# facebookresearch/iSDF

Measured on NVIDIA H100. Metric: train ray-samples/sec, higher is better.
Workload: dtype bf16x3 (bf16 hi/lo split, fp32 accumulate; weight-gradient operands single bf16)

## Files before the change

include/isdf_b200.h:

```cpp
#ifndef ISDF_B200_H_
#define ISDF_B200_H_

#include <stdint.h>

#ifdef __cplusplus
extern "C" {
#endif

typedef struct isdfb_ctx isdfb_ctx;

typedef enum {
  ISDFB_OK = 0,
  ISDFB_ERR_ARG = -1,
  ISDFB_ERR_CUDA = -2,
  ISDFB_ERR_CAPACITY = -3,
  ISDFB_ERR_STATE = -4
} isdfb_status;

typedef enum {
  ISDFB_PREC_FP32 = 0,
  ISDFB_PREC_BF16X3 = 1,
  ISDFB_PREC_BF16 = 2,
  ISDFB_PREC_BF16X3G = 3
} isdfb_precision;
// ... 24 lines not shown
} isdfb_loss_cfg;

typedef struct { float fx, fy, cx, cy; int32_t H, W; } isdfb_camera;

int isdfb_create(const isdfb_model_cfg* cfg, int device, isdfb_ctx** out);
int isdfb_destroy(isdfb_ctx* ctx);
const char* isdfb_last_error(const isdfb_ctx* ctx);
int64_t isdfb_param_count(const isdfb_ctx* ctx);
int32_t isdfb_embedding_size(const isdfb_ctx* ctx);
int64_t isdfb_launch_count(const isdfb_ctx* ctx);

int isdfb_pack_weights(isdfb_ctx* ctx, const float* params_flat, void* stream);

int isdfb_gather_rays(isdfb_ctx* ctx, const float* depth, const float* normals,
                      const int64_t* frame_map, int32_t normals_use_frame_map,
                      const int64_t* ib, const int64_t* ih, const int64_t* iw, int64_t n_rays,
                      const isdfb_camera* cam, float* depth_out, float* normal_out,
                      uint8_t* valid_out, void* stream);
int isdfb_sample_rays(isdfb_ctx* ctx, const float* T_WC , const int64_t* frame_map,
                      const int64_t* ib, const int64_t* ih, const int64_t* iw,
                      const float* dirs_C_in, const float* depth_sample, const float* far,
                      const float* near, const float* u_strat, const float* n_near,
                      const float* lin, int64_t n_rays, int32_t n_strat, int32_t n_surf,
                      const isdfb_camera* cam, float min_depth, float dist_behind,
                      float* pc , float* z_vals , float* dirs_C ,
                      float* T_WC_sample , void* stream);

int isdfb_sample_fused(isdfb_ctx* ctx, const float* depth, const float* normals, const float* T_WC,
                       const int64_t* frame_map, int32_t normals_use_frame_map, int32_t n_frames,
                       int32_t n_rays_per_frame, int32_t n_strat, int32_t n_surf, const isdfb_camera* cam,
                       float min_depth, float dist_behind, const float* lin, uint64_t seed, int64_t* ib, int64_t* ih,
                       int64_t* iw, float* pc, float* z_vals, float* dirs_C, float* T_WC_sample, float* depth_sample,
                       float* norm_sample, uint8_t* ray_valid, float* noise, float* inv_count, void* stream);

int isdfb_select_window(isdfb_ctx* ctx, const float* frame_avg_losses , int32_t n_frames,
                        int32_t window_size, uint64_t seed, int64_t* frame_map , void* stream);

int isdfb_ingest_normals(isdfb_ctx* ctx, const float* depth, const isdfb_camera* cam, float* normals,
                         void* stream);

int isdfb_pe_encode(isdfb_ctx* ctx, const float* x, int64_t n, float* out, void* stream);

int isdfb_mlp_forward(isdfb_ctx* ctx, const float* x, const float* noise, float noise_std,
                      int64_t n, float* sdf, void* stream);
int isdfb_mlp_forward_grad(isdfb_ctx* ctx, const float* x, const float* noise, float noise_std,
                           int64_t n, float* sdf, float* grad, void* stream);

int isdfb_mlp_forward_grid(isdfb_ctx* ctx, const float* lin , int32_t dim,
                           const float* scale , const float* transform ,
                           float* sdf , void* stream);

int isdfb_bounds_pc(isdfb_ctx* ctx, const float* pc, const float* z_vals, const float* depth_sample,
                    const uint8_t* ray_valid, int64_t n_rays, int32_t n_samples, float* bounds,
                    float* grad_vec, void* stream);

int isdfb_train_fwd_bwd(isdfb_ctx* ctx, const float* pc, const float* z_vals,
                        const float* depth_sample, const float* dirs_C, const float* T_WC_sample,
                        const float* norm_sample, const float* noise, const uint8_t* ray_valid,
                        int64_t n_rays, int32_t n_samples, const isdfb_loss_cfg* loss,
                        float* sdf, float* grad, float* loss_mat, float* loss_sums, void* stream);
int isdfb_zero_grad(isdfb_ctx* ctx, void* stream);
int isdfb_export_grads(isdfb_ctx* ctx, float* grads_flat, void* stream);

int isdfb_frame_bins(isdfb_ctx* ctx, const float* loss_mat, const uint8_t* ray_valid,
                     const int64_t* ib, const int64_t* ih, const int64_t* iw, int64_t n_rays,
                     int32_t n_samples, int32_t n_frames, int32_t H, int32_t W, int32_t factor,
                     float* loss_approx, float* frame_avg, void* stream);

int isdfb_step_finish(isdfb_ctx* ctx, const float* loss_mat, const uint8_t* ray_valid,
                      const int64_t* ib, const int64_t* ih, const int64_t* iw, int64_t n_rays,
                      int32_t n_samples, int32_t n_frames, int32_t H, int32_t W, int32_t factor,
                      float* loss_approx, float* frame_avg, const int64_t* frame_map, float* frame_avg_losses,
                      float* loss_sums, const float* inv_count, float* means_out, void* stream);

int isdfb_adamw(isdfb_ctx* ctx, float* params_flat, float* m, float* v, int64_t step, double lr,
                double beta1, double beta2, double eps, double weight_decay, float grad_scale,
                void* stream);
int isdfb_adamw_graph(isdfb_ctx* ctx, float* params_flat, float* m, float* v, double lr, double beta1,
                      double beta2, double eps, double weight_decay, float grad_scale, void* stream);
int isdfb_adamw_set_step(isdfb_ctx* ctx, int64_t step, void* stream);
int isdfb_grad_buffer(isdfb_ctx* ctx, float** ptr, int64_t* n_floats);

int isdfb_set_grad_exchange(isdfb_ctx* ctx, float* local0, float* local1, float* mcast0, float* mcast1,
                            int64_t n_floats);
int isdfb_select_grad_buffer(isdfb_ctx* ctx, int32_t which);
int isdfb_zero_grad_buffer(isdfb_ctx* ctx, int32_t which, void* stream);

int isdfb_mesh_count(isdfb_ctx* ctx, const float* sdf, int32_t dim, int64_t* n_verts ,
                     int64_t* n_faces , void* stream);
int isdfb_mesh_emit(isdfb_ctx* ctx, const float* sdf, int32_t dim, const float* scale ,
                    const float* transform , float* verts, int64_t cap_verts, int32_t* faces,
                    int64_t cap_faces, void* stream);

int isdfb_mesh_cloud(isdfb_ctx* ctx, const float* depth, const float* T_WC, int32_t n_frames, int32_t H, int32_t W,
                     int32_t H_vis, int32_t W_vis, float fx, float fy, float cx, float cy, float* cloud, float* box,
                     void* stream);
int isdfb_mesh_crop_count(isdfb_ctx* ctx, const float* cloud, int64_t n_cloud, float crop_dist, const float* verts,
                          int64_t n_verts, const int32_t* faces, int64_t n_faces, int64_t* n_verts_kept ,
                          int64_t* n_faces_kept , void* stream);
int isdfb_mesh_crop_emit(isdfb_ctx* ctx, const float* verts, int64_t n_verts, const int32_t* faces, int64_t n_faces,
                         float* verts_out, int64_t cap_verts, int32_t* faces_out, int64_t cap_faces, void* stream);

int isdfb_gt_sdf_sample(isdfb_ctx* ctx, const float* lattice, int32_t nx, int32_t ny, int32_t nz,
                        const double* origin , const double* spacing , const float* pts_f32,
                        const double* pts_f64, int64_t n, double fill, double* out, uint8_t* in_bounds, void* stream);

#define ISDFB_EVAL_NSTATS 17
int isdfb_sdf_error_stats(isdfb_ctx* ctx, const float* pred, const double* gt, const uint8_t* in_bounds,
                          const uint8_t* valid, int64_t n, double* out, void* stream);

int isdfb_points_visible(isdfb_ctx* ctx, const float* pts, int64_t n, const float* T_CW, const float* depth,
                         int32_t n_frames, int32_t H, int32_t W, float fx, float fy, float cx, float cy, float trunc,
                         uint8_t* vis, void* stream);

int isdfb_gt_sdf_grad(isdfb_ctx* ctx, const float* lattice, int32_t nx, int32_t ny, int32_t nz,
                      const double* origin , const double* spacing , const float* pts_f32,
                      const double* pts_f64, int64_t n, double delta, double* grad, uint8_t* valid, void* stream);

int isdfb_sdf_split_stats(isdfb_ctx* ctx, const float* pred, const double* gt, int64_t n, int64_t n_vox, double* out,
                          void* stream);

int isdfb_grad_cosdist(isdfb_ctx* ctx, const float* pred, const double* gt, const int64_t* gt_index, int64_t n,
                       double eps, double* out, void* stream);

#define ISDFB_CHOMP_MAX_EPS 4
int isdfb_chomp_costs(isdfb_ctx* ctx, const float* pred, const double* gt, const uint8_t* in_bounds, int64_t n,
                      const double* eps , int32_t n_eps, double* out, void* stream);

#define ISDFB_VOXELIZE_MAX_DEPTH 9
#define ISDFB_GT_SDF_MAX_DIM 16384
int isdfb_voxelize_count(isdfb_ctx* ctx, const double* verts, int64_t n_verts, const void* faces, int32_t faces_int64,
                         int64_t n_faces, double pitch, const double* origin , int64_t* box_lo ,
                         int64_t* box_dims , void* stream);
int isdfb_voxelize_emit(isdfb_ctx* ctx, const double* verts, int64_t n_verts, const void* faces, int32_t faces_int64,
                        int64_t n_faces, double pitch, const double* origin ,
                        const int64_t* box_lo , const int64_t* box_dims , uint8_t* box,
                        void* stream);
int isdfb_fill_holes(isdfb_ctx* ctx, uint8_t* box, int32_t nx, int32_t ny, int32_t nz, void* stream);
int isdfb_occupancy_sdf(isdfb_ctx* ctx, const uint8_t* occ, int32_t nx, int32_t ny, int32_t nz, double voxel_size,
                        double* sdf, void* stream);

int isdfb_profile_enable(isdfb_ctx* ctx, int32_t enable);
int isdfb_profile_read(isdfb_ctx* ctx, double* chain_ms, double* dw_ms, int64_t* n_chain, int64_t* n_dw);

int isdfb_debug_program(int32_t n_freqs, int32_t hidden, int32_t block, int32_t mode, int32_t* steps_out,
                        int32_t max_steps);

int isdfb_debug_mc_table(uint8_t* rows, int32_t* max_tris);

int isdfb_debug_buffers(isdfb_ctx* ctx, float** aux, int64_t* aux_stride_floats, void** dwl_hi,
                        void** dwl_lo, int64_t* dwl_stride_bytes, int32_t* n_aux, int32_t* n_dwl,
                        int64_t* tiles_cap, void** sig16);

#ifdef __cplusplus
}
#endif
#endif
```

isdf_b200/_lib.py:

```python
import ctypes as C
import os

_HERE = os.path.dirname(os.path.abspath(__file__))
LIB_PATH = os.path.join(_HERE, "lib", "libisdf_b200.so")

PREC_FP32, PREC_BF16X3, PREC_BF16, PREC_BF16X3G = 0, 1, 2, 3
PRECISIONS = {"fp32": PREC_FP32, "bf16x3": PREC_BF16X3, "bf16": PREC_BF16, "bf16x3g": PREC_BF16X3G}


class ModelCfg(C.Structure):
    _fields_ = [("n_freqs", C.c_int32), ("hidden", C.c_int32), ("block", C.c_int32),
                ("has_transform", C.c_int32), ("scale_input", C.c_float), ("scale_output", C.c_float),
                ("transform", C.c_float * 12), ("precision", C.c_int32), ("max_points", C.c_int32)]


class LossCfg(C.Structure):
    _fields_ = [("trunc_weight", C.c_float), ("trunc_distance", C.c_float), ("eik_weight", C.c_float),
                ("eik_apply_dist", C.c_float), ("grad_weight", C.c_float), ("orien_loss", C.c_int32),
                ("loss_type", C.c_int32), ("noise_std", C.c_float), ("inv_count", C.c_float),
                ("inv_count_dev", C.c_void_p), ("bounds_dev", C.c_void_p), ("grad_vec_dev", C.c_void_p)]


class Camera(C.Structure):
    _fields_ = [("fx", C.c_float), ("fy", C.c_float), ("cx", C.c_float), ("cy", C.c_float),
                ("H", C.c_int32), ("W", C.c_int32)]


P = C.c_void_p
I64 = C.c_int64
I32 = C.c_int32
F = C.c_float
D = C.c_double

SIGNATURES = {
    "isdfb_create": (C.c_int, [C.POINTER(ModelCfg), C.c_int, C.POINTER(P)]),
    "isdfb_destroy": (C.c_int, [P]),
    "isdfb_last_error": (C.c_char_p, [P]),
    "isdfb_param_count": (I64, [P]),
    "isdfb_embedding_size": (I32, [P]),
    "isdfb_launch_count": (I64, [P]),
    "isdfb_pack_weights": (C.c_int, [P, P, P]),
    "isdfb_gather_rays": (C.c_int, [P, P, P, P, I32, P, P, P, I64, C.POINTER(Camera), P, P, P, P]),
    "isdfb_sample_rays": (C.c_int, [P, P, P, P, P, P, P, P, P, P, P, P, P, I64, I32, I32, C.POINTER(Camera), F, F,
                                    P, P, P, P, P]),
    "isdfb_sample_fused": (C.c_int, [P, P, P, P, P, I32, I32, I32, I32, I32, C.POINTER(Camera), F, F, P, C.c_uint64,
                                     P, P, P, P, P, P, P, P, P, P, P, P, P]),
    "isdfb_ingest_normals": (C.c_int, [P, P, C.POINTER(Camera), P, P]),
    "isdfb_pe_encode": (C.c_int, [P, P, I64, P, P]),
    "isdfb_mlp_forward": (C.c_int, [P, P, P, F, I64, P, P]),
    "isdfb_mlp_forward_grad": (C.c_int, [P, P, P, F, I64, P, P, P]),
    "isdfb_mlp_forward_grid": (C.c_int, [P, P, I32, C.POINTER(F), C.POINTER(F), P, P]),
    "isdfb_bounds_pc": (C.c_int, [P, P, P, P, P, I64, I32, P, P, P]),
    "isdfb_train_fwd_bwd": (C.c_int, [P, P, P, P, P, P, P, P, P, I64, I32, C.POINTER(LossCfg), P, P, P, P, P]),
    "isdfb_zero_grad": (C.c_int, [P, P]),
    "isdfb_set_grad_exchange": (C.c_int, [P, P, P, P, P, I64]),
    "isdfb_select_grad_buffer": (C.c_int, [P, I32]),
    "isdfb_zero_grad_buffer": (C.c_int, [P, I32, P]),
    "isdfb_export_grads": (C.c_int, [P, P, P]),
    "isdfb_frame_bins": (C.c_int, [P, P, P, P, P, P, I64, I32, I32, I32, I32, I32, P, P, P]),
    "isdfb_step_finish": (C.c_int, [P, P, P, P, P, P, I64, I32, I32, I32, I32, I32, P, P, P, P, P, P, P, P]),
    "isdfb_select_window": (C.c_int, [P, P, I32, I32, C.c_uint64, P, P]),
    "isdfb_adamw": (C.c_int, [P, P, P, P, I64, D, D, D, D, D, F, P]),
    "isdfb_adamw_graph": (C.c_int, [P, P, P, P, D, D, D, D, D, F, P]),
    "isdfb_adamw_set_step": (C.c_int, [P, I64, P]),
    "isdfb_grad_buffer": (C.c_int, [P, C.POINTER(P), C.POINTER(I64)]),
    "isdfb_mesh_count": (C.c_int, [P, P, I32, C.POINTER(I64), C.POINTER(I64), P]),
    "isdfb_mesh_emit": (C.c_int, [P, P, I32, C.POINTER(F), C.POINTER(F), P, I64, P, I64, P]),
    "isdfb_mesh_cloud": (C.c_int, [P, P, P, I32, I32, I32, I32, I32, F, F, F, F, P, P, P]),
    "isdfb_mesh_crop_count": (C.c_int, [P, P, I64, F, P, I64, P, I64, C.POINTER(I64), C.POINTER(I64), P]),
    "isdfb_mesh_crop_emit": (C.c_int, [P, P, I64, P, I64, P, I64, P, I64, P]),
    "isdfb_gt_sdf_sample": (C.c_int, [P, P, I32, I32, I32, C.POINTER(C.c_double), C.POINTER(C.c_double), P, P, I64,
                                      C.c_double, P, P, P]),
    "isdfb_sdf_error_stats": (C.c_int, [P, P, P, P, P, I64, P, P]),
    "isdfb_points_visible": (C.c_int, [P, P, I64, P, P, I32, I32, I32, F, F, F, F, F, P, P]),
    "isdfb_gt_sdf_grad": (C.c_int, [P, P, I32, I32, I32, C.POINTER(C.c_double), C.POINTER(C.c_double), P, P, I64,
                                    C.c_double, P, P, P]),
    "isdfb_sdf_split_stats": (C.c_int, [P, P, P, I64, I64, P, P]),
    "isdfb_grad_cosdist": (C.c_int, [P, P, P, P, I64, C.c_double, P, P]),
    "isdfb_chomp_costs": (C.c_int, [P, P, P, P, I64, C.POINTER(C.c_double), I32, P, P]),
    "isdfb_voxelize_count": (C.c_int, [P, P, I64, P, I32, I64, D, C.POINTER(D), C.POINTER(I64), C.POINTER(I64), P]),
    "isdfb_voxelize_emit": (C.c_int, [P, P, I64, P, I32, I64, D, C.POINTER(D), C.POINTER(I64), C.POINTER(I64), P, P]),
    "isdfb_fill_holes": (C.c_int, [P, P, I32, I32, I32, P]),
    "isdfb_occupancy_sdf": (C.c_int, [P, P, I32, I32, I32, D, P, P]),
    "isdfb_profile_enable": (C.c_int, [P, I32]),
    "isdfb_profile_read": (C.c_int, [P, C.POINTER(C.c_double), C.POINTER(C.c_double), C.POINTER(I64), C.POINTER(I64)]),
    "isdfb_debug_program": (C.c_int, [I32, I32, I32, I32, C.POINTER(I32), I32]),
    "isdfb_debug_mc_table": (C.c_int, [C.POINTER(C.c_uint8), C.POINTER(I32)]),
    "isdfb_debug_buffers": (C.c_int, [P, C.POINTER(P), C.POINTER(I64), C.POINTER(P), C.POINTER(P), C.POINTER(I64),
                                      C.POINTER(I32), C.POINTER(I32), C.POINTER(I64), C.POINTER(P)]),
}

_lib = None


def load():
    global _lib
    if _lib is not None:
        return _lib
    if not os.path.exists(LIB_PATH):
        raise RuntimeError(
            "isdf_b200: CUDA library %s not found. Build it with `python -c 'import __graft_entry__ as g; "
            "g.build()'` (nvcc, sm_90a). There is no CPU fallback." % LIB_PATH)
    lib = C.CDLL(LIB_PATH)
    for name, (res, args) in SIGNATURES.items():
        fn = getattr(lib, name)
        fn.restype = res
        fn.argtypes = args
    _lib = lib
    return lib


ERR_ARG, ERR_CUDA, ERR_CAPACITY, ERR_STATE = -1, -2, -3, -4


class IsdfbError(RuntimeError):

    def __init__(self, msg, rc=None):
        super().__init__(msg)
        self.rc = rc


def check(rc, ctx=None):
    if rc != 0:
        msg = load().isdfb_last_error(ctx)
        raise IsdfbError("isdf_b200 error %d: %s" % (rc, msg.decode() if msg else "?"), rc)
```

isdf_b200/csrc/tc_dw.cu:

```cuda
#include "tc_path.cuh"

#define DW_CONS_WG 2
#define DW_THREADS (128 * (1 + DW_CONS_WG))
#define DW_CONS_REGS 224
#define DW_PROD_REGS 56

template <int kPasses> struct DwCfg {
  static constexpr int kXBytes = 4096 * (kPasses == 3 ? 2 : 1);
  static constexpr int kYBytes = 8192 * (kPasses == 3 ? 2 : 1);
  static constexpr int kStageBytes = kXBytes + kYBytes;
  static constexpr int kStages = (kPasses == 3) ? 8 : 12;
  static constexpr int kSmem = kStages * kStageBytes + 512 + 256;
};

struct DwSmemTail {
  uint64_t full[12], empty[12];
};

template <int kPasses>
__global__ void __launch_bounds__(DW_THREADS, 1) tc_dw_kernel(const __grid_constant__ TcDwArgs args) {
  using Cfg = DwCfg<kPasses>;
  extern __shared__ __align__(1024) uint8_t smem[];
  uint8_t* ring = smem;
  uint8_t* ones = smem + Cfg::kStages * Cfg::kStageBytes;
  DwSmemTail* tail = reinterpret_cast<DwSmemTail*>(ones + 512);
  const int warp = threadIdx.x >> 5, lane = threadIdx.x & 31;

  const int job_id = blockIdx.x % args.n_jobs;
  const int split = blockIdx.x / args.n_jobs;
  const int n_splits = ((int)gridDim.x - 1 - job_id) / args.n_jobs + 1;
  const int my_tiles = (args.n_tiles > split) ? (args.n_tiles - 1 - split) / n_splits + 1 : 0;
  const TcDwJob& job = args.jobs[job_id];

  if (threadIdx.x < 128) reinterpret_cast<uint32_t*>(ones)[threadIdx.x] = 0x3F803F80u;
  if (threadIdx.x == 0) {
    for (int i = 0; i < Cfg::kStages; ++i) { mbar_init(smem_u32(&tail->full[i]), 1); mbar_init(smem_u32(&tail->empty[i]), DW_CONS_WG); }
    mbar_fence_init();
  }
  fence_proxy_async_smem();
  __syncthreads();

  bool has_main = false, has_db = false, has_dw = false;
  for (int pi = 0; pi < job.n_pairs; ++pi) {
    has_main |= job.pair[pi].y_arr >= 0;
    has_db |= job.pair[pi].ones == 1;
    has_dw |= job.pair[pi].ones == 2;
  }

  if (warp < 4) {
    reg_dec<DW_PROD_REGS>();
    if (warp == 0 && elect_one()) {
      uint32_t j = 0;
      for (int it = 0; it < my_tiles; ++it) {
        const size_t tile_off = (size_t)(args.tile0 + split + it * n_splits) * TC_DWL_TILE_BYTES;
        for (int pi = 0; pi < job.n_pairs; ++pi) {
          const TcDwPair pr = job.pair[pi];
          const size_t xo = (size_t)pr.x_arr * args.dwl_stride + tile_off + (size_t)job.half * 4096;
          const size_t yo = (size_t)(pr.y_arr < 0 ? 0 : pr.y_arr) * args.dwl_stride + tile_off;
          const uint32_t bytes = Cfg::kXBytes + (pr.y_arr >= 0 ? Cfg::kYBytes : 0);
          for (int ks = 0; ks < 8; ++ks, ++j) {
            const uint32_t stage = j % Cfg::kStages, ph = (j / Cfg::kStages) & 1;
            mbar_wait(smem_u32(&tail->empty[stage]), ph ^ 1);
            const uint32_t bar = smem_u32(&tail->full[stage]);
            const uint32_t dst = smem_u32(ring + stage * Cfg::kStageBytes);
            mbar_arrive_expect_tx(bar, bytes);
            bulk_g2s(dst, args.dwl_hi + xo + (size_t)ks * 8192, 4096, bar);
            if (kPasses == 3) bulk_g2s(dst + 4096, args.dwl_lo + xo + (size_t)ks * 8192, 4096, bar);
            if (pr.y_arr >= 0) {
              bulk_g2s(dst + Cfg::kXBytes, args.dwl_hi + yo + (size_t)ks * 8192, 8192, bar);
              if (kPasses == 3) bulk_g2s(dst + Cfg::kXBytes + 8192, args.dwl_lo + yo + (size_t)ks * 8192, 8192, bar);
            }
          }
        }
      }
    }
  } else {
    reg_inc<DW_CONS_REGS>();
    const int g = (warp >> 2) - 1, wq = warp & 3, q4 = lane & 3;
    const bool leader = (threadIdx.x & 127) == 0;
    float d_main[128], d_db[8], d_dw[8];
#pragma unroll
    for (int r = 0; r < 128; ++r) d_main[r] = 0.f;
#pragma unroll
    for (int r = 0; r < 8; ++r) { d_db[r] = 0.f; d_dw[r] = 0.f; }
    uint32_t j = 0, acc_main = 0, acc_db = 0, acc_dw = 0;
    const uint64_t b_ones = gmma_desc(smem_u32(ones), 128, 256);
    wgmma_fence();
    for (int it = 0; it < my_tiles; ++it) {
      for (int pi = 0; pi < job.n_pairs; ++pi) {
        const TcDwPair pr = job.pair[pi];
#pragma unroll 1
        for (int ks = 0; ks < 8; ++ks, ++j) {
          const uint32_t stage = j % Cfg::kStages, ph = (j / Cfg::kStages) & 1;
          mbar_wait(smem_u32(&tail->full[stage]), ph);
          const uint32_t base = smem_u32(ring + stage * Cfg::kStageBytes);
          const uint64_t ah = gmma_desc(base + 2048u * g, 128, 256);
          const uint64_t al = gmma_desc(base + 4096 + 2048u * g, 128, 256);
          if (pr.y_arr >= 0) {
            const uint64_t bh = gmma_desc(base + Cfg::kXBytes, 128, 256);
            wgmma_m64n256k16<1, 1>(d_main, ah, bh, acc_main);
            if (kPasses == 3) {
              wgmma_m64n256k16<1, 1>(d_main, al, bh, 1);
              wgmma_m64n256k16<1, 1>(d_main, ah, gmma_desc(base + Cfg::kXBytes + 8192, 128, 256), 1);
            }
            acc_main = 1;
          }
          if (pr.ones == 1) {
            wgmma_m64n16k16<1, 1>(d_db, ah, b_ones, acc_db);
            if (kPasses == 3) wgmma_m64n16k16<1, 1>(d_db, al, b_ones, 1);
            acc_db = 1;
          } else if (pr.ones == 2) {
            wgmma_m64n16k16<1, 1>(d_dw, ah, b_ones, acc_dw);
            if (kPasses == 3) wgmma_m64n16k16<1, 1>(d_dw, al, b_ones, 1);
            acc_dw = 1;
          }
          wgmma_commit();
          if (j > 0) {
            wgmma_wait<1>();
            if (leader) mbar_arrive(smem_u32(&tail->empty[(j - 1) % Cfg::kStages]));
          }
        }
      }
    }
    wgmma_wait<0>();
    wgmma_fence_operands<128>(d_main);
    wgmma_fence_operands<8>(d_db);
    wgmma_fence_operands<8>(d_dw);
    if (my_tiles > 0) {
      const int r0 = job.half * 128 + 64 * g + 16 * wq + (lane >> 2);
      if (has_main) {
#pragma unroll
        for (int rh = 0; rh < 2; ++rh) {
          float* grow = args.g_packed + job.g_off + (size_t)(r0 + 8 * rh) * job.ld;
          if (job.perm_half > 0) {
#pragma unroll
            for (int i = 0; i < 32; ++i)
#pragma unroll
              for (int e = 0; e < 2; ++e) {
                const int nat = pe_nat_col(job.col0 + 8 * i + 2 * q4 + e, job.perm_half);
                if (nat < job.ld) grad_add(grow + nat, d_main[4 * i + 2 * rh + e], 0);
              }
          } else {
#pragma unroll
            for (int i = 0; i < 32; ++i) grad_add2(grow + 8 * i + 2 * q4, d_main[4 * i + 2 * rh], d_main[4 * i + 2 * rh + 1]);
          }
        }
      }
      if (q4 == 0) {
#pragma unroll
        for (int rh = 0; rh < 2; ++rh) {
          if (has_db) grad_add(args.g_packed + job.db_off + r0 + 8 * rh, d_db[2 * rh], 0);
          if (has_dw) grad_add(args.g_packed + args.wout_off + r0 + 8 * rh, args.scale_output * d_dw[2 * rh], 0);
        }
      }
    }
    if (args.g_mc) {
      __shared__ int s_last;
      const int t = threadIdx.x - 128;
      __threadfence();
      named_bar_sync(3, 128 * DW_CONS_WG);
      if (t == 0) {
        const int prev = (my_tiles > 0) ? atomicAdd(args.counters + job_id, 1) : -1;
        s_last = (prev == args.expect[job_id] - 1) ? 1 : 0;
        if (s_last) args.counters[job_id] = 0;
      }
      named_bar_sync(3, 128 * DW_CONS_WG);
      if (s_last) {
        __threadfence();
        const size_t base = job.g_off + (size_t)(job.half * 128) * job.ld;
        if (has_main) {
          float4* src = reinterpret_cast<float4*>(args.g_packed + base) + t;
          float* dst = args.g_mc_out + base + (size_t)t * 4;
#pragma unroll 1
          for (int it = 0; it < 32; it += 8) {
            float4 r[8];
#pragma unroll
            for (int u = 0; u < 8; ++u) r[u] = __ldcg(src + (size_t)(it + u) * 256);
#pragma unroll
            for (int u = 0; u < 8; ++u) {
              grad_add4(dst + (size_t)(it + u) * 1024, r[u].x, r[u].y, r[u].z, r[u].w, 1);
              __stcg(src + (size_t)(it + u) * 256, make_float4(0.f, 0.f, 0.f, 0.f));
            }
          }
        }
        if (t < 128) {
          const int row = job.half * 128 + t;
          if (has_db) {
            float* p = args.g_packed + job.db_off + row;
            grad_add(args.g_mc_out + job.db_off + row, __ldcg(p), 1);
            __stcg(p, 0.f);
          }
          if (has_dw) {
            float* p = args.g_packed + args.wout_off + row;
            grad_add(args.g_mc_out + args.wout_off + row, __ldcg(p), 1);
            __stcg(p, 0.f);
          }
        }
      }
    }
  }
}

int tc_dw_launch(isdfb_ctx* ctx, const TcDwArgs& args, int passes, int grid, cudaStream_t st) {
  if (grid < args.n_jobs)
    ISDFB_FAIL(ctx, ISDFB_ERR_ARG, "weight-gradient launch of %d CTAs for %d jobs: every job needs a CTA", grid,
               args.n_jobs);
  if (passes == 3) {
    tc_dw_kernel<3><<<grid, DW_THREADS, DwCfg<3>::kSmem, st>>>(args);
  } else {
    tc_dw_kernel<1><<<grid, DW_THREADS, DwCfg<1>::kSmem, st>>>(args);
  }
  ISDFB_LAUNCHED(ctx);
  ISDFB_CUDA_OK(ctx, cudaGetLastError());
  return ISDFB_OK;
}

int tc_dw_init(isdfb_ctx* ctx) {
  ISDFB_CUDA_OK(ctx, cudaFuncSetAttribute(tc_dw_kernel<3>, cudaFuncAttributeMaxDynamicSharedMemorySize, DwCfg<3>::kSmem));
  ISDFB_CUDA_OK(ctx, cudaFuncSetAttribute(tc_dw_kernel<1>, cudaFuncAttributeMaxDynamicSharedMemorySize, DwCfg<1>::kSmem));
  return ISDFB_OK;
}
```

isdf_b200/csrc/tc_path.cu:

```cuda
#include "tc_path.cuh"
#include <new>

static TcStep& add_step(TcChainArgs& a, int unit, int orient, int epi, int layer, int aux = 0) {
  TcStep& s = a.steps[a.n_steps++];
  s.unit = unit; s.orient = orient; s.epi = epi; s.layer = (int16_t)layer; s.aux = (int16_t)aux;
  s.addp = -1; s.flags = 0; s.peh = 0; s.eh = 0;
  return s;
}

enum { PART_CAT_S1 = 0, PART_CAT_S2 = 1, PART_CAT_S3 = 2, PART_CAT_S2_H1 = 3, PART_L0_S1 = 4, PART_L0_S3 = 5 };

static void build_program(const ModelLayout& lay, int mode, int NE, TcChainArgs& a) {
  const int L = lay.L, ic = lay.block + 1, UE = L, U0B = L + 1, UEB = L + 2;
  a.n_steps = 0;
  add_step(a, UE, 0, EPI_RAW, 0, PART_CAT_S1);
  if (NE == 2) {
    TcStep& r = add_step(a, 0, 0, EPI_RAW, 0, PART_L0_S1);
    r.flags = STF_PE_E; r.peh = 1;
    add_step(a, UEB, 0, EPI_RAW, 0, PART_CAT_S1).flags = STF_RAW_ADD;
  }
  for (int l = 0; l < L; ++l) {
    TcStep& t = add_step(a, (l == 0 && NE == 2) ? U0B : l, 0, l == L - 1 ? EPI_S1_LAST : EPI_S1, l);
    if (l == 0 && NE == 2) t.addp = PART_L0_S1;
    if (l == ic) t.addp = PART_CAT_S1;
// ... 212 lines not shown

static inline int wave1_dw_grid(const TcState* tc, int rest) {
  const int free_sms = tc->num_sms - rest;
  return free_sms > tc->dw.n_jobs ? free_sms : tc->dw.n_jobs;
}

static int tc_forward_impl(isdfb_ctx* ctx, const float* x, const float* noise, float noise_std, int64_t n, float* sdf,
                           float* grad, cudaStream_t st, const TcGrid* grid) {
  TcState* tc = reinterpret_cast<TcState*>(ctx->tc);
  for (int64_t p0 = 0; p0 < n; p0 += ctx->cap) {
    const int64_t nc = (n - p0 < ctx->cap) ? (n - p0) : ctx->cap;
    TcChainArgs a = tc->proto[grad ? TC_MODE_FWD_GRAD : TC_MODE_FWD];
    if (grid) a.grid = *grid;
    a.n_points = nc;
    a.n_tiles = (int)((nc + TC_TILE - 1) / TC_TILE);
    a.p0 = p0;
    a.x = x ? x + p0 * 3 : nullptr;
    a.noise = noise ? noise + p0 : nullptr;
    a.noise_std = noise_std;
    a.sdf_out = sdf + p0;
    a.g_out = grad ? grad + p0 * 3 : nullptr;
    const int n_cta = a.n_tiles < tc->num_sms ? a.n_tiles : tc->num_sms;
    const int pi = prof_begin(tc, st);
    int rc = tc_chain_launch(ctx, a, passes_of(ctx), n_cta, st);
    if (rc) return rc;
    prof_mark(tc, pi, 1, st);
  }
  return ISDFB_OK;
}

int tc_forward(isdfb_ctx* ctx, const float* x, const float* noise, float noise_std, int64_t n, float* sdf,
               float* grad, cudaStream_t st) {
  return tc_forward_impl(ctx, x, noise, noise_std, n, sdf, grad, st, nullptr);
}

int tc_forward_grid(isdfb_ctx* ctx, const float* lin, int dim, const float* scale, const float* transform, float* sdf,
                    cudaStream_t st) {
  if ((int64_t)dim * dim * dim >= (1LL << 32))
    ISDFB_FAIL(ctx, ISDFB_ERR_ARG, "grid dim %d too large for the tensor-core path (dim^3 must be < 2^32)", dim);
  TcGrid g;
  memset(&g, 0, sizeof(g));
  g.lin = lin; g.dim = dim;
  for (int i = 0; i < 3; ++i) g.scale[i] = scale ? scale[i] : 1.f;
  g.has_transform = transform ? 1 : 0;
  if (transform)
    for (int r = 0; r < 3; ++r) {
      for (int c = 0; c < 3; ++c) g.R[r * 3 + c] = transform[r * 4 + c];
      g.t[r] = transform[r * 4 + 3];
    }
  return tc_forward_impl(ctx, nullptr, nullptr, 0.f, (int64_t)dim * dim * dim, sdf, nullptr, st, &g);
}

int tc_train(isdfb_ctx* ctx, const float* pc, const float* z_vals, const float* depth_sample, const float* dirs_C,
             const float* T_WC_sample, const float* norm_sample, const float* noise, const uint8_t* ray_valid,
             int64_t n_rays, int32_t S, const isdfb_loss_cfg* loss, float* sdf, float* grad, float* loss_mat,
             float* loss_sums, cudaStream_t st) {
  TcState* tc = reinterpret_cast<TcState*>(ctx->tc);
  const int64_t n = n_rays * S;
  if (n >= (1LL << 32))
    ISDFB_FAIL(ctx, ISDFB_ERR_ARG, "%lld samples per step exceed the tensor-core path's 2^32", (long long)n);
  const bool two_wave_ok = !tc->profiling;
  int32_t expect[TC_MAX_JOBS] = {0};
  if (ctx->g_xchg) {
    auto plan = [&](int grid, int tiles) {
      for (int j = 0; j < tc->dw.n_jobs; ++j) {
        const int n_splits = (grid - 1 - j) / tc->dw.n_jobs + 1;
        expect[j] += n_splits < tiles ? n_splits : tiles;
      }
    };
    for (int64_t p0 = 0; p0 < n; p0 += ctx->cap) {
      const int64_t nc = (n - p0 < ctx->cap) ? (n - p0) : ctx->cap;
      const int tiles = (int)((nc + TC_TILE - 1) / TC_TILE);
      if (tiles > tc->num_sms && tiles < 2 * tc->num_sms && two_wave_ok) {
        const int rest = tiles - tc->num_sms;
        plan(wave1_dw_grid(tc, rest), tc->num_sms);
        plan(tc->num_sms, rest);
      } else {
        plan(tc->num_sms, tiles);
      }
    }
  }
  for (int64_t p0 = 0; p0 < n; p0 += ctx->cap) {
    const int64_t nc = (n - p0 < ctx->cap) ? (n - p0) : ctx->cap;
    TcChainArgs a = tc->proto[TC_MODE_TRAIN];
    a.n_points = nc;
    a.n_tiles = (int)((nc + TC_TILE - 1) / TC_TILE);
    a.p0 = p0;
    a.S = S;
    a.loss = *loss;
    a.x = pc + p0 * 3;
    a.noise = noise ? noise + p0 : nullptr;
    a.noise_std = loss->noise_std;
    a.sdf_out = sdf + p0;
    a.g_out = grad ? grad + p0 * 3 : nullptr;
    a.z_vals = z_vals; a.depth = depth_sample; a.dirs_C = dirs_C; a.T_WC = T_WC_sample; a.normals = norm_sample;
    a.ray_valid = ray_valid;
    a.loss_mat = loss_mat;
    a.loss_sums = loss_sums;
    a.g_packed = ctx->g_xchg ? ctx->g_mc[ctx->g_sel] : ctx->g_packed;
    a.g_mc = ctx->g_xchg ? 1 : 0;
    const int total_tiles = a.n_tiles;
    const int pi = prof_begin(tc, st);
    TcDwArgs d = tc->dw;
    d.g_mc = ctx->g_xchg ? 1 : 0;
    d.g_packed = ctx->g_xchg ? ctx->g_own : ctx->g_packed;
    d.g_mc_out = ctx->g_xchg ? ctx->g_mc[ctx->g_sel] : nullptr;
    d.counters = tc->dw_counters;
    for (int j = 0; j < TC_MAX_JOBS; ++j) d.expect[j] = expect[j];
    int rc;
    if (total_tiles > tc->num_sms && total_tiles < 2 * tc->num_sms && two_wave_ok) {
      a.tile0 = 0; a.n_tiles = tc->num_sms;
      rc = tc_chain_launch(ctx, a, passes_of(ctx), tc->num_sms, st);
      if (rc) return rc;
      ISDFB_CUDA_OK(ctx, cudaEventRecord(tc->ev_fork, st));
      ISDFB_CUDA_OK(ctx, cudaStreamWaitEvent(tc->side, tc->ev_fork, 0));
      d.tile0 = 0; d.n_tiles = tc->num_sms;
      const int rest = total_tiles - tc->num_sms;
      rc = tc_dw_launch(ctx, d, dw_passes_of(ctx), wave1_dw_grid(tc, rest), tc->side);
      if (rc) return rc;
      ISDFB_CUDA_OK(ctx, cudaEventRecord(tc->ev_join, tc->side));
      a.tile0 = tc->num_sms; a.n_tiles = rest;
      rc = tc_chain_launch(ctx, a, passes_of(ctx), rest, st);
      if (rc) return rc;
      ISDFB_CUDA_OK(ctx, cudaStreamWaitEvent(st, tc->ev_join, 0));
      d.tile0 = tc->num_sms; d.n_tiles = rest;
      rc = tc_dw_launch(ctx, d, dw_passes_of(ctx), tc->num_sms, st);
      if (rc) return rc;
    } else {
      const int grid = a.n_tiles < tc->num_sms ? a.n_tiles : tc->num_sms;
      rc = tc_chain_launch(ctx, a, passes_of(ctx), grid, st);
      if (rc) return rc;
      prof_mark(tc, pi, 1, st);
      d.tile0 = 0; d.n_tiles = total_tiles;
      rc = tc_dw_launch(ctx, d, dw_passes_of(ctx), tc->num_sms, st);
      if (rc) return rc;
      prof_mark(tc, pi, 2, st);
    }
  }
  return ISDFB_OK;
}

extern "C" int isdfb_debug_buffers(isdfb_ctx* ctx, float** aux, int64_t* aux_stride_floats, void** dwl_hi,
                                   void** dwl_lo, int64_t* dwl_stride_bytes, int32_t* n_aux, int32_t* n_dwl,
                                   int64_t* tiles_cap, void** sig16) {
  if (!ctx) return ISDFB_ERR_ARG;
  TcState* tc = reinterpret_cast<TcState*>(ctx->tc);
  if (!tc) ISDFB_FAIL(ctx, ISDFB_ERR_STATE, "no tensor-core state (fp32 path)");
  *aux = tc->aux; *aux_stride_floats = (int64_t)tc->aux_stride;
  *dwl_hi = tc->dwl_hi; *dwl_lo = tc->dwl_lo; *dwl_stride_bytes = (int64_t)tc->dwl_stride;
  *n_aux = tc->n_aux; *n_dwl = tc->n_dwl; *tiles_cap = tc->tiles_cap; *sig16 = tc->sig16;
  return ISDFB_OK;
}

extern "C" int isdfb_profile_enable(isdfb_ctx* ctx, int32_t enable) {
  if (!ctx) return ISDFB_ERR_ARG;
  TcState* tc = reinterpret_cast<TcState*>(ctx->tc);
  if (!tc) ISDFB_FAIL(ctx, ISDFB_ERR_STATE, "kernel timing is available on the tensor-core path only");
  tc->profiling = enable != 0;
  tc->n_ev = 0;
  return ISDFB_OK;
}

extern "C" int isdfb_profile_read(isdfb_ctx* ctx, double* chain_ms, double* dw_ms, int64_t* n_chain, int64_t* n_dw) {
  if (!ctx || !chain_ms || !dw_ms || !n_chain || !n_dw) return ISDFB_ERR_ARG;
  TcState* tc = reinterpret_cast<TcState*>(ctx->tc);
  if (!tc) ISDFB_FAIL(ctx, ISDFB_ERR_STATE, "kernel timing is available on the tensor-core path only");
  ISDFB_CUDA_OK(ctx, cudaSetDevice(ctx->device));
  *chain_ms = *dw_ms = 0.0; *n_chain = *n_dw = 0;
  for (int i = 0; i < tc->n_ev; ++i) {
    const int k = tc->ev_kind[i];
    if (k < 1) continue;
    float ms = 0.f;
    ISDFB_CUDA_OK(ctx, cudaEventSynchronize(tc->ev[i][k]));
    ISDFB_CUDA_OK(ctx, cudaEventElapsedTime(&ms, tc->ev[i][0], tc->ev[i][1]));
    *chain_ms += ms; ++*n_chain;
    if (k == 2) {
      ISDFB_CUDA_OK(ctx, cudaEventElapsedTime(&ms, tc->ev[i][1], tc->ev[i][2]));
      *dw_ms += ms; ++*n_dw;
    }
  }
  tc->n_ev = 0;
  return ISDFB_OK;
}
```

isdf_b200/engine.py:

```python
import ctypes as C

import torch

from . import _lib

F32, F64, I32, I64, U8 = torch.float32, torch.float64, torch.int32, torch.int64, torch.uint8
_SMALL_INTS = (torch.uint8, torch.int8, torch.int16, torch.int32)


def _ptr(t):
    return C.c_void_p(t.data_ptr()) if t is not None else C.c_void_p(0)


def _shape_ok(t, shape, rows):
    if isinstance(shape, int):
        ok = t.numel() == shape
    elif shape is None:
        ok = True
    else:
        want = shape[1:] if shape[0] is ... else shape
        got = t.shape[max(t.dim() - len(want), 0):] if shape[0] is ... else t.shape
        ok = len(got) == len(want) and all(w is None or w == g for w, g in zip(want, got))
    return ok and (rows == 0 or (t.dim() > 0 and t.shape[0] >= rows))

# ... 338 lines not shown
        return box

    def occupancy_sdf(self, occ, voxel_size):
        occ = self._arg(occ, "occ", U8, (None, None, None))
        sdf = torch.empty(occ.shape, dtype=torch.float64, device=self.device)
        self._ck(self.lib.isdfb_occupancy_sdf(self._ctx, _ptr(occ), *occ.shape, float(voxel_size), _ptr(sdf),
                                              self._stream()))
        return sdf

    def bounds_pc(self, pc, z_vals, depth_sample, ray_valid=None):
        dev = self.device
        z_vals = self._arg(z_vals, "z_vals", F32, (None, None))
        R, S = z_vals.shape
        pc, depth_sample = self._arg(pc, "pc", F32, (R, S, 3)), self._arg(depth_sample, "depth_sample", F32, (R,))
        ray_valid = self._arg(ray_valid, "ray_valid", U8, (R,))
        bounds = torch.empty(R, S, dtype=torch.float32, device=dev)
        vec = torch.empty(R, S, 3, dtype=torch.float32, device=dev)
        self._ck(self.lib.isdfb_bounds_pc(self._ctx, _ptr(pc), _ptr(z_vals), _ptr(depth_sample), _ptr(ray_valid),
                                          R, S, _ptr(bounds), _ptr(vec), self._stream()))
        return bounds, vec

    def train_fwd_bwd(self, pc, z_vals, depth_sample, dirs_C, T_WC_sample, norm_sample, noise, loss_cfg,
                      ray_valid=None, want_grad=True, loss_sums=None):
        dev = self.device
        pc = self._arg(pc, "pc", F32, (None, None, 3))
        R, S = pc.shape[0], pc.shape[1]
        z_vals = self._arg(z_vals, "z_vals", F32, (R, S))
        depth_sample = self._arg(depth_sample, "depth_sample", F32, (R,))
        dirs_C = self._arg(dirs_C, "dirs_C_sample", F32, (R, 3))
        T_WC_sample = self._arg(T_WC_sample, "T_WC_sample", F32, (R, 4, 4))
        norm_sample = self._arg(norm_sample, "norm_sample", F32, (R, 3))
        noise, ray_valid = self._arg(noise, "noise", F32, (R, S)), self._arg(ray_valid, "ray_valid", U8, (R,))
        self._arg(loss_cfg.bounds, "bounds", F32, (R, S), as_is=True)
        self._arg(loss_cfg.grad_vec, "grad_vec", F32, (R, S, 3), as_is=True)
        self._arg(loss_cfg.inv_count_tensor, "inv_count_dev", F32, (None,), rows=1, as_is=True)
        if loss_sums is None:
            loss_sums = torch.zeros(4, dtype=torch.float32, device=dev)
        loss_sums = self._arg(loss_sums, "loss_sums", F32, (4,), as_is=True)
        sdf = torch.empty(R, S, dtype=torch.float32, device=dev)
        g = torch.empty(R, S, 3, dtype=torch.float32, device=dev) if want_grad else None
        loss_mat = torch.empty(R, S, dtype=torch.float32, device=dev)
        self._ck(self.lib.isdfb_train_fwd_bwd(self._ctx, _ptr(pc), _ptr(z_vals), _ptr(depth_sample), _ptr(dirs_C),
                                              _ptr(T_WC_sample), _ptr(norm_sample), _ptr(noise), _ptr(ray_valid),
                                              R, S, C.byref(loss_cfg), _ptr(sdf), _ptr(g), _ptr(loss_mat),
                                              _ptr(loss_sums), self._stream()))
        return sdf, g, loss_mat, loss_sums

    def zero_grad(self):
        self._ck(self.lib.isdfb_zero_grad(self._ctx, self._stream()))

    def set_grad_exchange(self, local0, local1, mcast0, mcast1, n_floats):
        self._ck(self.lib.isdfb_set_grad_exchange(self._ctx, C.c_void_p(local0), C.c_void_p(local1), C.c_void_p(mcast0),
                                                  C.c_void_p(mcast1), int(n_floats)))

    def select_grad_buffer(self, which):
        self._ck(self.lib.isdfb_select_grad_buffer(self._ctx, int(which)))

    def zero_grad_buffer(self, which):
        self._ck(self.lib.isdfb_zero_grad_buffer(self._ctx, int(which), self._stream()))

    def export_grads(self, out=None):
        if out is None:
            out = torch.empty(self.n_params, dtype=torch.float32, device=self.device)
        out = self._arg(out, "out", F32, self.n_params, as_is=True)
        self._ck(self.lib.isdfb_export_grads(self._ctx, _ptr(out), self._stream()))
        return out

    def grad_buffer(self):
        p, n = C.c_void_p(), C.c_int64()
        self._ck(self.lib.isdfb_grad_buffer(self._ctx, C.byref(p), C.byref(n)))
        return _DevView(p.value, n.value, self.device).tensor

    def frame_bins(self, loss_mat, ib, ih, iw, n_frames, H, W, factor=8, ray_valid=None):
        dev = self.device
        loss_mat = self._arg(loss_mat, "loss_mat", F32, (None, None))
        R, S = loss_mat.shape
        ib, ih, iw = (self._arg(ib, "indices_b", I64, (R,)), self._arg(ih, "indices_h", I64, (R,)),
                      self._arg(iw, "indices_w", I64, (R,)))
        ray_valid = self._arg(ray_valid, "ray_valid", U8, (R,))
        approx = torch.empty(n_frames, factor, factor, dtype=torch.float32, device=dev)
        favg = torch.empty(n_frames, dtype=torch.float32, device=dev)
        self._ck(self.lib.isdfb_frame_bins(self._ctx, _ptr(loss_mat), _ptr(ray_valid), _ptr(ib), _ptr(ih), _ptr(iw),
                                           R, S, int(n_frames), int(H), int(W), int(factor), _ptr(approx),
                                           _ptr(favg), self._stream()))
        return approx, favg

    def step_finish(self, loss_mat, ib, ih, iw, n_frames, H, W, factor, ray_valid, frame_map, frame_avg_losses,
                    loss_sums, inv_count, means_out):
        dev = self.device
        loss_mat = self._arg(loss_mat, "loss_mat", F32, (None, None), as_is=True)
        R, S = loss_mat.shape
        ib = self._arg(ib, "indices_b", I64, (R,), as_is=True)
        ih, iw = self._arg(ih, "indices_h", I64, (R,), as_is=True), self._arg(iw, "indices_w", I64, (R,), as_is=True)
        ray_valid = self._arg(ray_valid, "ray_valid", U8, (R,))
        frame_map = self._arg(frame_map, "frame_map", I64, (None,), rows=n_frames, as_is=True)
        frame_avg_losses = self._arg(frame_avg_losses, "frame_avg_losses", F32, (None,), rows=n_frames, as_is=True)
        loss_sums = self._arg(loss_sums, "loss_sums", F32, (4,), as_is=True)
        inv_count = self._arg(inv_count, "inv_count", F32, (None,), rows=1, as_is=True)
        means_out = self._arg(means_out, "means_out", F32, (4,), as_is=True)
        approx = torch.empty(n_frames, factor, factor, dtype=torch.float32, device=dev)
        favg = torch.empty(n_frames, dtype=torch.float32, device=dev)
        self._ck(self.lib.isdfb_step_finish(self._ctx, _ptr(loss_mat), _ptr(ray_valid), _ptr(ib), _ptr(ih), _ptr(iw), R, S,
                                            int(n_frames), int(H), int(W), int(factor), _ptr(approx), _ptr(favg),
                                            _ptr(frame_map), _ptr(frame_avg_losses), _ptr(loss_sums), _ptr(inv_count),
                                            _ptr(means_out), self._stream()))
        return approx, favg

    def select_window(self, frame_avg_losses, n_frames, window_size, seed, out=None):
        w = self._arg(frame_avg_losses, "frame_avg_losses", F32, (None,), rows=n_frames)
        if out is None:
            out = torch.empty(window_size, dtype=torch.int64, device=self.device)
        out = self._arg(out, "out", I64, (window_size,), as_is=True)
        self._ck(self.lib.isdfb_select_window(self._ctx, _ptr(w), int(n_frames), int(window_size),
                                              C.c_uint64(int(seed) & (2 ** 64 - 1)), _ptr(out), self._stream()))
        return out

    def _adamw_state(self, params, m, v):
        n = self.n_params
        return (_ptr(self._arg(params, "params", F32, n, as_is=True)),
                _ptr(self._arg(m, "exp_avg", F32, n, as_is=True)), _ptr(self._arg(v, "exp_avg_sq", F32, n, as_is=True)))

    def adamw(self, params, m, v, step, lr, beta1=0.9, beta2=0.999, eps=1e-8, weight_decay=0.01, grad_scale=1.0):
        self._ck(self.lib.isdfb_adamw(self._ctx, *self._adamw_state(params, m, v), int(step), float(lr), float(beta1),
                                      float(beta2), float(eps), float(weight_decay), float(grad_scale),
                                      self._stream()))

    def adamw_graph(self, params, m, v, lr, beta1=0.9, beta2=0.999, eps=1e-8, weight_decay=0.01, grad_scale=1.0):
        self._ck(self.lib.isdfb_adamw_graph(self._ctx, *self._adamw_state(params, m, v), float(lr), float(beta1),
                                            float(beta2), float(eps), float(weight_decay), float(grad_scale),
                                            self._stream()))

    def adamw_set_step(self, step):
        self._ck(self.lib.isdfb_adamw_set_step(self._ctx, int(step), self._stream()))

    def profile(self, enable):
        self._ck(self.lib.isdfb_profile_enable(self._ctx, 1 if enable else 0))

    def profile_read(self):
        c, d = C.c_double(), C.c_double()
        nc, nd = C.c_int64(), C.c_int64()
        self._ck(self.lib.isdfb_profile_read(self._ctx, C.byref(c), C.byref(d), C.byref(nc), C.byref(nd)))
        return dict(chain_ms=c.value, dw_ms=d.value, n_chain=nc.value, n_dw=nd.value)

    def debug_buffers(self):
        aux, dhi, dlo, sg = C.c_void_p(), C.c_void_p(), C.c_void_p(), C.c_void_p()
        a_st, d_st, tiles = C.c_int64(), C.c_int64(), C.c_int64()
        n_aux, n_dwl = C.c_int32(), C.c_int32()
        self._ck(self.lib.isdfb_debug_buffers(self._ctx, C.byref(aux), C.byref(a_st), C.byref(dhi), C.byref(dlo),
                                              C.byref(d_st), C.byref(n_aux), C.byref(n_dwl), C.byref(tiles), C.byref(sg)))
        return dict(aux=aux.value or 0, aux_stride_floats=a_st.value, dwl_hi=dhi.value or 0, dwl_lo=dlo.value or 0,
                    dwl_stride_bytes=d_st.value, n_aux=n_aux.value, n_dwl=n_dwl.value, tiles=tiles.value,
                    sig16=sg.value or 0)


class _DevView:

    def __init__(self, ptr, n, device):
        self.__cuda_array_interface__ = {"shape": (n,), "typestr": "<f4", "data": (ptr, False), "version": 2}
        self.tensor = torch.as_tensor(self, device=device)


def make_loss_cfg(trunc_weight, trunc_distance, eik_weight, eik_apply_dist, grad_weight, orien_loss, loss_type,
                  noise_std, inv_count, inv_count_dev=None, bounds=None, grad_vec=None):
    lc = _lib.LossCfg()
    lc.trunc_weight, lc.trunc_distance = float(trunc_weight), float(trunc_distance)
    lc.eik_weight, lc.eik_apply_dist = float(eik_weight), float(eik_apply_dist)
    lc.grad_weight = float(grad_weight)
    lc.orien_loss = 1 if orien_loss else 0
    if loss_type not in ("L1", "L2"):
        raise ValueError("Must be L1 or L2")
    lc.loss_type = 1 if loss_type == "L1" else 2
    lc.noise_std = float(noise_std or 0.0)
    lc.inv_count = float(inv_count)
    if (bounds is None) != (grad_vec is None):
        raise ValueError("bounds and grad_vec (the outputs of Engine.bounds_pc) go together")
    lc.inv_count_tensor, lc.bounds, lc.grad_vec = inv_count_dev, bounds, grad_vec
    lc.inv_count_dev, lc.bounds_dev, lc.grad_vec_dev = [None if t is None else t.data_ptr()
                                                        for t in (inv_count_dev, bounds, grad_vec)]
    return lc


def make_camera(fx, fy, cx, cy, H, W):
    cam = _lib.Camera()
    cam.fx, cam.fy, cam.cx, cam.cy, cam.H, cam.W = float(fx), float(fy), float(cx), float(cy), int(H), int(W)
    return cam


def pe_nat_col(c, half):
    if half <= 0:
        return c
    if c < 2 * half:
        return 3 + (c >> 1) + (c & 1) * half
    if c < 2 * half + 3:
        return c - 2 * half
    return c


class SideState:

    def __init__(self, engine, n_points):
        b = engine.debug_buffers()
        self.L = 2 * engine.block + 2
        self.E = engine.embedding_size
        self.NE = 2 if self.E > 256 else 1
        self.half = 21 * engine.n_freqs
        self.lean = engine.precision == "bf16x3g"
        self.n = int(n_points)
        self.tiles = -(-self.n // 128)
        self.rows = 128 * self.tiles
        cap, d_st, L, NE = b["tiles"], b["dwl_stride_bytes"], self.L, self.NE
        n_part = 6 if NE == 2 else 3
        self.arr_part, self.arr_e32, self.arr_hlast, self.arr_zb2 = 0, n_part, n_part + NE, n_part + NE + 1
        self.arr_yh, self.arr_ya, self.arr_xd, self.arr_xz, self.arr_v = 0, L, 2 * L, 3 * L, 4 * L
        self.arr_yh_e1, self.arr_ya_e1 = 4 * L + 1, 4 * L + 2
        assert b["n_aux"] == n_part + NE + 1 + (0 if self.lean else L), b
        assert b["n_dwl"] == 4 * L + 1 + (2 if NE == 2 else 0), b
        assert self.tiles <= cap
        dev = engine.device
        self._engine = engine
        self.has_lo = bool(b["dwl_lo"])
        self._aux = _DevView(b["aux"], b["aux_stride_floats"] * b["n_aux"], dev).tensor.view(b["n_aux"], cap, 64, 128, 4)

        def bytes16(ptr, n_arr):
            return _DevView(ptr, d_st * n_arr // 4, dev).tensor.view(torch.int16)

        self._hi = bytes16(b["dwl_hi"], b["n_dwl"]).view(b["n_dwl"], cap, 8, 32, 16, 8)
        self._lo = bytes16(b["dwl_lo"], b["n_dwl"]).view(b["n_dwl"], cap, 8, 32, 16, 8) if b["dwl_lo"] else None
        n_sig = L * (2 if self.lean else 1)
        self._sig = bytes16(b["sig16"], n_sig).view(n_sig, cap, 32, 128, 8)
        idx = [pe_nat_col(c, self.half) for c in range(256 * NE)]
        self._nat_src = torch.tensor([c for c in range(256 * NE) if idx[c] < self.E], device=dev)
        self._nat_dst = torch.tensor([idx[c] for c in range(256 * NE) if idx[c] < self.E], device=dev)

    def aux(self, arr):
        return self._aux[arr, :self.tiles].permute(0, 2, 1, 3).reshape(self.rows, 256).clone()

    def dwl(self, arr, part="hi"):
        src = self._hi if part == "hi" else self._lo
        if src is None:
            raise ValueError("no %s image in %s mode" % (part, "bf16x3g" if self.lean else "this"))
        x = src[arr, :self.tiles].permute(0, 1, 3, 2, 4).reshape(self.rows, 256).contiguous()
        return x.view(torch.bfloat16).float()

    def sigma_code(self, l):
        return self._sig[l, :self.tiles].permute(0, 2, 1, 3).reshape(self.rows, 256).to(torch.int32) & 0xFFFF

    def sigma(self, l):
        return self.sigma_code(l).float() / 65535.0

    def zbar2(self, l):
        if not self.lean:
            return self.aux(self.arr_zb2 + l)
        x = self._sig[self.L + l, :self.tiles].permute(0, 2, 1, 3).reshape(self.rows, 256).contiguous()
        return x.view(torch.bfloat16).float()

    def natural(self, halves):
        x = torch.cat(halves, dim=1)
        out = torch.zeros(x.shape[0], self.E, dtype=x.dtype, device=x.device)
        out[:, self._nat_dst] = x[:, self._nat_src]
        return out

    def e32(self):
        return self.natural([self.aux(self.arr_e32 + h) for h in range(self.NE)])

    def operand(self, name, l=0, part="hi"):
        if name == "v":
            return self.dwl(self.arr_v, part)
        base = dict(yh=self.arr_yh, ya=self.arr_ya, xd=self.arr_xd, xz=self.arr_xz)[name]
        if name in ("yh", "ya") and l == 0:
            halves = [self.dwl(base, part)]
            if self.NE == 2:
                halves.append(self.dwl(self.arr_yh_e1 if name == "yh" else self.arr_ya_e1, part))
            return self.natural(halves)
        return self.dwl(base + l, part)


def debug_state(engine, n_points):
    return SideState(engine, n_points)
```

Before: 22.94 million.

## Size dW ring stages from a byte budget and merge bias/output-weight accumulators

New measurement: 23.74 million, median of 6. 1.03x the previous value.

```diff
diff --git a/include/isdf_b200.h b/include/isdf_b200.h
--- a/include/isdf_b200.h
+++ b/include/isdf_b200.h
@@ -200,6 +200,8 @@
                         void** dwl_lo, int64_t* dwl_stride_bytes, int32_t* n_aux, int32_t* n_dwl,
                         int64_t* tiles_cap, void** sig16);
 
+int isdfb_debug_dw_launch(isdfb_ctx* ctx, int32_t tile0, int32_t n_tiles, int32_t grid, void* stream);
+
 #ifdef __cplusplus
 }
 #endif
diff --git a/isdf_b200/_lib.py b/isdf_b200/_lib.py
--- a/isdf_b200/_lib.py
+++ b/isdf_b200/_lib.py
@@ -86,6 +86,7 @@
     "isdfb_profile_read": (C.c_int, [P, C.POINTER(C.c_double), C.POINTER(C.c_double), C.POINTER(I64), C.POINTER(I64)]),
     "isdfb_debug_program": (C.c_int, [I32, I32, I32, I32, C.POINTER(I32), I32]),
     "isdfb_debug_mc_table": (C.c_int, [C.POINTER(C.c_uint8), C.POINTER(I32)]),
+    "isdfb_debug_dw_launch": (C.c_int, [P, I32, I32, I32, P]),
     "isdfb_debug_buffers": (C.c_int, [P, C.POINTER(P), C.POINTER(I64), C.POINTER(P), C.POINTER(P), C.POINTER(I64),
                                       C.POINTER(I32), C.POINTER(I32), C.POINTER(I64), C.POINTER(P)]),
 }
diff --git a/isdf_b200/csrc/tc_dw.cu b/isdf_b200/csrc/tc_dw.cu
--- a/isdf_b200/csrc/tc_dw.cu
+++ b/isdf_b200/csrc/tc_dw.cu
@@ -5,16 +5,18 @@
 #define DW_CONS_REGS 224
 #define DW_PROD_REGS 56
 
+#define DW_RING_BYTES (216 * 1024)
 template <int kPasses> struct DwCfg {
   static constexpr int kXBytes = 4096 * (kPasses == 3 ? 2 : 1);
   static constexpr int kYBytes = 8192 * (kPasses == 3 ? 2 : 1);
   static constexpr int kStageBytes = kXBytes + kYBytes;
-  static constexpr int kStages = (kPasses == 3) ? 8 : 12;
-  static constexpr int kSmem = kStages * kStageBytes + 512 + 256;
+  static constexpr int kStages = DW_RING_BYTES / kStageBytes;
+  static constexpr int kSmem = kStages * kStageBytes + 1024 + 512;
 };
+#define DW_MAX_STAGES (DW_RING_BYTES / 12288)
 
 struct DwSmemTail {
-  uint64_t full[12], empty[12];
+  uint64_t full[DW_MAX_STAGES], empty[DW_MAX_STAGES];
 };
 
 template <int kPasses>
@@ -23,7 +25,7 @@
   extern __shared__ __align__(1024) uint8_t smem[];
   uint8_t* ring = smem;
   uint8_t* ones = smem + Cfg::kStages * Cfg::kStageBytes;
-  DwSmemTail* tail = reinterpret_cast<DwSmemTail*>(ones + 512);
+  DwSmemTail* tail = reinterpret_cast<DwSmemTail*>(ones + 1024);
   const int warp = threadIdx.x >> 5, lane = threadIdx.x & 31;
 
   const int job_id = blockIdx.x % args.n_jobs;
@@ -32,7 +34,8 @@
   const int my_tiles = (args.n_tiles > split) ? (args.n_tiles - 1 - split) / n_splits + 1 : 0;
   const TcDwJob& job = args.jobs[job_id];
 
-  if (threadIdx.x < 128) reinterpret_cast<uint32_t*>(ones)[threadIdx.x] = 0x3F803F80u;
+  if (threadIdx.x < 256)
+    reinterpret_cast<uint32_t*>(ones)[threadIdx.x] = ((threadIdx.x >> 6) & 1) == (threadIdx.x >> 7) ? 0x3F803F80u : 0u;
   if (threadIdx.x == 0) {
     for (int i = 0; i < Cfg::kStages; ++i) { mbar_init(smem_u32(&tail->full[i]), 1); mbar_init(smem_u32(&tail->empty[i]), DW_CONS_WG); }
     mbar_fence_init();
@@ -78,13 +81,14 @@
     reg_inc<DW_CONS_REGS>();
     const int g = (warp >> 2) - 1, wq = warp & 3, q4 = lane & 3;
     const bool leader = (threadIdx.x & 127) == 0;
-    float d_main[128], d_db[8], d_dw[8];
+    float d_main[128], d_cs[8];
 #pragma unroll
     for (int r = 0; r < 128; ++r) d_main[r] = 0.f;
 #pragma unroll
-    for (int r = 0; r < 8; ++r) { d_db[r] = 0.f; d_dw[r] = 0.f; }
-    uint32_t j = 0, acc_main = 0, acc_db = 0, acc_dw = 0;
-    const uint64_t b_ones = gmma_desc(smem_u32(ones), 128, 256);
+    for (int r = 0; r < 8; ++r) d_cs[r] = 0.f;
+    uint32_t j = 0, acc_main = 0, acc_cs = 0;
+    const uint64_t b_ones_db = gmma_desc(smem_u32(ones), 128, 256);
+    const uint64_t b_ones_dw = gmma_desc(smem_u32(ones + 512), 128, 256);
     wgmma_fence();
     for (int it = 0; it < my_tiles; ++it) {
       for (int pi = 0; pi < job.n_pairs; ++pi) {
@@ -105,14 +109,11 @@
             }
             acc_main = 1;
           }
-          if (pr.ones == 1) {
-            wgmma_m64n16k16<1, 1>(d_db, ah, b_ones, acc_db);
-            if (kPasses == 3) wgmma_m64n16k16<1, 1>(d_db, al, b_ones, 1);
-            acc_db = 1;
-          } else if (pr.ones == 2) {
-            wgmma_m64n16k16<1, 1>(d_dw, ah, b_ones, acc_dw);
-            if (kPasses == 3) wgmma_m64n16k16<1, 1>(d_dw, al, b_ones, 1);
-            acc_dw = 1;
+          if (pr.ones != 0) {
+            const uint64_t b_ones = pr.ones == 1 ? b_ones_db : b_ones_dw;
+            wgmma_m64n16k16<1, 1>(d_cs, ah, b_ones, acc_cs);
+            if (kPasses == 3) wgmma_m64n16k16<1, 1>(d_cs, al, b_ones, 1);
+            acc_cs = 1;
           }
           wgmma_commit();
           if (j > 0) {
@@ -124,8 +125,7 @@
     }
     wgmma_wait<0>();
     wgmma_fence_operands<128>(d_main);
-    wgmma_fence_operands<8>(d_db);
-    wgmma_fence_operands<8>(d_dw);
+    wgmma_fence_operands<8>(d_cs);
     if (my_tiles > 0) {
       const int r0 = job.half * 128 + 64 * g + 16 * wq + (lane >> 2);
       if (has_main) {
@@ -149,8 +149,8 @@
       if (q4 == 0) {
 #pragma unroll
         for (int rh = 0; rh < 2; ++rh) {
-          if (has_db) grad_add(args.g_packed + job.db_off + r0 + 8 * rh, d_db[2 * rh], 0);
-          if (has_dw) grad_add(args.g_packed + args.wout_off + r0 + 8 * rh, args.scale_output * d_dw[2 * rh], 0);
+          if (has_db) grad_add(args.g_packed + job.db_off + r0 + 8 * rh, d_cs[2 * rh], 0);
+          if (has_dw) grad_add(args.g_packed + args.wout_off + r0 + 8 * rh, args.scale_output * d_cs[4 + 2 * rh], 0);
         }
       }
     }
diff --git a/isdf_b200/csrc/tc_path.cu b/isdf_b200/csrc/tc_path.cu
--- a/isdf_b200/csrc/tc_path.cu
+++ b/isdf_b200/csrc/tc_path.cu
@@ -388,6 +388,23 @@
   return ISDFB_OK;
 }
 
+extern "C" int isdfb_debug_dw_launch(isdfb_ctx* ctx, int32_t tile0, int32_t n_tiles, int32_t grid, void* stream) {
+  if (!ctx) return ISDFB_ERR_ARG;
+  TcState* tc = reinterpret_cast<TcState*>(ctx->tc);
+  if (!tc) ISDFB_FAIL(ctx, ISDFB_ERR_STATE, "no tensor-core state (fp32 path)");
+  if (tile0 < 0 || n_tiles < 1 || (int64_t)tile0 + n_tiles > tc->tiles_cap || grid < 1)
+    ISDFB_FAIL(ctx, ISDFB_ERR_ARG, "weight-gradient launch of tiles [%d, %d) on %d CTAs (%lld tiles allocated)", tile0,
+               tile0 + n_tiles, grid, (long long)tc->tiles_cap);
+  ISDFB_CUDA_OK(ctx, cudaSetDevice(ctx->device));
+  TcDwArgs d = tc->dw;
+  d.g_packed = ctx->g_packed;
+  d.g_mc = 0;
+  d.g_mc_out = nullptr;
+  d.counters = tc->dw_counters;
+  d.tile0 = tile0; d.n_tiles = n_tiles;
+  return tc_dw_launch(ctx, d, dw_passes_of(ctx), grid, (cudaStream_t)stream);
+}
+
 extern "C" int isdfb_profile_enable(isdfb_ctx* ctx, int32_t enable) {
   if (!ctx) return ISDFB_ERR_ARG;
   TcState* tc = reinterpret_cast<TcState*>(ctx->tc);
diff --git a/isdf_b200/engine.py b/isdf_b200/engine.py
--- a/isdf_b200/engine.py
+++ b/isdf_b200/engine.py
@@ -514,6 +514,9 @@
                     dwl_stride_bytes=d_st.value, n_aux=n_aux.value, n_dwl=n_dwl.value, tiles=tiles.value,
                     sig16=sg.value or 0)
 
+    def debug_dw_launch(self, tile0, n_tiles, grid):
+        self._ck(self.lib.isdfb_debug_dw_launch(self._ctx, int(tile0), int(n_tiles), int(grid), self._stream()))
+
 
 class _DevView:
 
```
